# lambdaclass/lambda_elliptic_curves

Measured on AMD Instinct MI355X. Metric: NTT elems/sec (Stark252 radix-2, 2^24, forward, bit-exact vs CPU: see 'bit_exact') [+ MSM G1 point-adds/sec under 'msm'], higher is better.
Workload: dtype u32x8 (256-bit Montgomery, 32-bit limbs)

## Files before the change

lambda_elliptic_curves_amd/csrc/ntt256.hip:

```cpp
#include <stdlib.h>
#include <vector>
#include "internal.h"
#include "ntt_kernels.cuh"
#include "pass_run.h"

namespace lw {

template <class Fn>
static int with_field(int field, Fn f) {
    if (field == LW_FIELD_STARK252) return f(Stark252{});
    if (field == LW_FIELD_BLS12_381_FR) return f(Fr381{});
    set_error("field %d has no 256-bit NTT", field);
    return LW_ERR_BAD_ARG;
}

template <class F>
static Fe<F> host_root_of_unity(uint32_t order, bool inverse) {
    if (order == 0) return Fe<F>::one();
    Fe<F> g;
    for (int i = 0; i < F::N; i++) g.v[i] = F::root(i);
    g = fe_to_mont<F>(g);
    for (uint32_t i = 0; i < F::TWO_ADICITY - order; i++) g = fe_sqr<F>(g);
    if (inverse) g = fe_inv<F>(g);
    return g;
}

template <class F>
static int upload_power_tables(const Fe<F> &base, uint32_t hbits, uint64_t hi_count, DeviceBuf &lo, DeviceBuf &hi,
                               const Fe<F> *hi_scale = nullptr) {
    const uint64_t lo_count = 1ull << hbits;
    std::vector<uint32_t> hl(lo_count * 8), hh(hi_count * 8);
    Fe<F> acc = Fe<F>::one();
    for (uint64_t i = 0; i < lo_count; i++) {
        for (int k = 0; k < 8; k++) hl[i * 8 + k] = acc.v[k];
        acc = fe_mul<F>(acc, base);
    }
    Fe<F> step = acc;
    acc = hi_scale ? *hi_scale : Fe<F>::one();
    for (uint64_t i = 0; i < hi_count; i++) {
        for (int k = 0; k < 8; k++) hh[i * 8 + k] = acc.v[k];
        acc = fe_mul<F>(acc, step);
    }
    if (lo.ensure(lo_count * 32) || hi.ensure(hi_count * 32)) return LW_ERR_ALLOC;
    LW_HIP_CHECK(hipMemcpy(lo.p, hl.data(), lo_count * 32, hipMemcpyHostToDevice), LW_ERR_LAUNCH);
    LW_HIP_CHECK(hipMemcpy(hi.p, hh.data(), hi_count * 32, hipMemcpyHostToDevice), LW_ERR_LAUNCH);
    return LW_OK;
}

template <class F>
static int ensure_twiddles(Context &c, int field, lw_dir_t dir, uint32_t log2n, hipStream_t stream) {
    TwiddleTable &t = c.tw[field][dir];
    DeviceBuf lo, hi;
    const int rc = ensure_twiddle_table(c, t, log2n, F::TWO_ADICITY, 32, stream, [&](uint32_t L) {
        const uint32_t bits = L - 1, hbits = (bits + 1) / 2;
        const uint64_t count = 1ull << bits;
        const int urc = upload_power_tables<F>(host_root_of_unity<F>(L, dir == LW_DIR_INVERSE), hbits, 1ull << (bits - hbits), lo, hi);
        if (urc) return urc;
        hipLaunchKernelGGL((twiddle_fill_kernel<F>), dim3((uint32_t)((count + 255) / 256)), dim3(256), 0, stream, (uint4 *)t.buf.p,
                           (const uint4 *)lo.p, (const uint4 *)hi.p, bits, hbits, count);
        return (int)LW_OK;
    });
    lo.release();
    hi.release();
    return rc;
}

template <class F>
static void launch_pass(bool last, dim3 grid, hipStream_t stream, const NttPassParams &p) {
    const bool extra = p.cos_in || p.cos_out || p.scale;
    bool wl = last && p.r >= 6;
    uint32_t ws = 0;
    for (uint32_t st = 0; st < p.nsteps && wl; st++)
        if ((1u << (p.r + p.logC - p.k[st])) != (uint32_t)NTT_THREADS) wl = false;
    if (wl)
        for (uint32_t st = 1; st < p.nsteps; st++)
            if (p.k[st] == p.k[st - 1] && (1u << (p.r - p.k[st])) <= 64u) ws |= 1u << st;
    NttPassParams q = p;
    q.wave_sync = ws;
#define LW_LAUNCH_PASS(LASTV, EXTRAV)                                                                                          \
    do {                                                                                                                       \
        if (fx == 8 && wl) hipLaunchKernelGGL((ntt_pass_kernel<F, LASTV, EXTRAV, LASTV, FXOK ? 8 : 0>), grid, dim3(NTT_THREADS), 0, stream, q);   \
        else if (fx == 8) hipLaunchKernelGGL((ntt_pass_kernel<F, LASTV, EXTRAV, false, FXOK ? 8 : 0>), grid, dim3(NTT_THREADS), 0, stream, q);   \
        else if (fx == 6 && !wl) hipLaunchKernelGGL((ntt_pass_kernel<F, LASTV, EXTRAV, false, FXOK ? 6 : 0>), grid, dim3(NTT_THREADS), 0, stream, q);   \
        else if (fx == 7 && !wl) hipLaunchKernelGGL((ntt_pass_kernel<F, LASTV, EXTRAV, false, FXOK ? 7 : 0>), grid, dim3(NTT_THREADS), 0, stream, q);   \
        else if (wl) hipLaunchKernelGGL((ntt_pass_kernel<F, LASTV, EXTRAV, LASTV>), grid, dim3(NTT_THREADS), 0, stream, q);  \
        else hipLaunchKernelGGL((ntt_pass_kernel<F, LASTV, EXTRAV, false>), grid, dim3(NTT_THREADS), 0, stream, q);      \
    } while (0)
    constexpr bool FXOK = NTT_TILE == 2048 && NTT_THREADS == 512;
    int fx = 0;
    if (FXOK && p.r == 8 && p.logC == 3 && p.nsteps == 4 && p.k[0] == 2 && p.k[1] == 2 && p.k[2] == 2 && p.k[3] == 2) fx = 8;
    if (FXOK && p.r == 7 && p.logC == 4 && p.nsteps == 4 && p.k[0] == 2 && p.k[1] == 2 && p.k[2] == 2 && p.k[3] == 1) fx = 7;
    if (FXOK && p.r == 6 && p.logC == 5 && p.nsteps == 3 && p.k[0] == 2 && p.k[1] == 2 && p.k[2] == 2) fx = 6;
    if (last) {
        if (extra) LW_LAUNCH_PASS(true, true);
        else LW_LAUNCH_PASS(true, false);
    } else {
        if (extra) LW_LAUNCH_PASS(false, true);
        else LW_LAUNCH_PASS(false, false);
    }
#undef LW_LAUNCH_PASS
}

template <class F>
static int power_tables(Context &c, int field, int slot, const uint32_t *base_words, bool invert, uint32_t hbits,
                        uint32_t hi_bits, hipStream_t stream, const uint4 **lo, const uint4 **hi, bool fold_ninv = false) {
    CosetCache &cc = c.coset[slot];
    bool hit = cc.valid && cc.field == field && cc.hbits == hbits && cc.hi_bits == hi_bits && cc.inverse == invert &&
               cc.fold_ninv == fold_ninv;
    for (int i = 0; i < 8 && hit; i++) hit = cc.words[i] == base_words[i];
    if (!hit) {
        Fe<F> b;
        for (int i = 0; i < 8; i++) b.v[i] = base_words[i];
        if (b.is_zero()) {
            set_error("coset offset is zero");
            return LW_ERR_INV_ZERO;
        }
        if (invert) b = fe_inv<F>(b);
        const uint64_t lo_count = 1ull << hbits, hi_count = 1ull << hi_bits;
        if (cc.lo.ensure(lo_count * 32) || cc.hi.ensure(hi_count * 32)) return LW_ERR_ALLOC;
        FeWords8 bw{}, sw{};
        for (int i = 0; i < 8; i++) bw.w[i] = b.v[i];
        if (fold_ninv) {
            const Fe<F> ninv = fe_inv<F>(fe_from_u64<F>(1ull << (hbits + hi_bits)));
            for (int i = 0; i < 8; i++) sw.w[i] = ninv.v[i];
        }
        hipLaunchKernelGGL((power_tables_kernel<F>), dim3((uint32_t)((lo_count + hi_count + 255) / 256)), dim3(256), 0, stream, (uint4 *)cc.lo.p,
                           (uint4 *)cc.hi.p, bw, hbits, hi_count, sw, fold_ninv ? 1 : 0);
        LW_HIP_CHECK(hipGetLastError(), LW_ERR_LAUNCH);
        cc.valid = true;
        cc.fold_ninv = fold_ninv;
        cc.field = field;
        cc.hbits = hbits;
        cc.hi_bits = hi_bits;
        cc.inverse = invert;
        for (int i = 0; i < 8; i++) cc.words[i] = base_words[i];
    }
    *lo = (const uint4 *)cc.lo.p;
    *hi = (const uint4 *)cc.hi.p;
    return LW_OK;
}

template <class F>
static int ntt256_run(Context &c, int field, lw_dir_t dir, const void *d_in, void *d_out, uint32_t log2n,
                      uint32_t batch, uint64_t stride, const uint32_t *coset_words, hipStream_t stream, uint32_t in_log2) {
    const uint64_t n = 1ull << log2n;
    if (stride == 0) stride = n;
    uint32_t skip = 0;
    if (dir == LW_DIR_FORWARD && in_log2 >= 1 && in_log2 < log2n) skip = log2n - in_log2;
    const uint64_t in_mask = skip ? ((1ull << in_log2) - 1) : ~0ull;
    if (log2n == 0) {
        if (d_in != d_out)
            LW_HIP_CHECK(hipMemcpy2DAsync(d_out, stride * 32, d_in, stride * 32, 32, batch, hipMemcpyDeviceToDevice, stream),
                         LW_ERR_LAUNCH);
        return LW_OK;
    }
    int rc = ensure_twiddles<F>(c, field, dir, log2n, stream);
    if (rc) return rc;
    const uint4 *tw = (const uint4 *)c.tw[field][dir].buf.p;

    const NttPlan pl = plan_passes(log2n, log2n, skip, NTT_TILE_LOG, NTT_KMAX, true);
    if ((pl.npass > 1 || d_in == d_out) && c.scratch.ensure((size_t)n * batch * 32)) return LW_ERR_ALLOC;
    c.timings.scratch_bytes = c.scratch.bytes;

    const uint4 *cos_lo = nullptr, *cos_hi = nullptr;
    const uint32_t cos_hbits = (log2n + 1) / 2;
    if (coset_words) {
        const bool inv = dir == LW_DIR_INVERSE;
        rc = power_tables<F>(c, field, inv ? 1 : 0, coset_words, inv, cos_hbits, log2n - cos_hbits, stream, &cos_lo, &cos_hi, inv);
        if (rc) return rc;
    }
    return run_passes(c, schedule_passes(pl, false, d_in == d_out), log2n, d_in, skip ? (1ull << in_log2) : stride, d_out, stride, batch,
                      c.scratch.p, 32, stream, [&](const PassStep &st, const void *in, void *out, uint64_t in_stride, uint64_t out_stride, dim3 grid) {
        NttPassParams p{};
        p.tw = tw;
        p.lazy_in = (F::LAZY && st.i > 0) ? 1 : 0;
        p.in_mask = st.first ? in_mask : ~0ull;
        p.cos_lo = cos_lo;
        p.cos_hi = cos_hi;
        p.cos_hbits = cos_hbits;
        p.cos_in = (coset_words && dir == LW_DIR_FORWARD && st.first) ? 1 : 0;
        p.cos_out = (coset_words && dir == LW_DIR_INVERSE && st.last) ? 1 : 0;
        p.L = log2n;
        p.s0 = st.s0;
        p.r = st.r;
        p.logC = st.logC;
        p.nsteps = st.nsteps;
        for (uint32_t q = 0; q < p.nsteps; q++) p.k[q] = st.k[q];
        p.in = (const uint4 *)in;
        p.in_batch_stride = in_stride;
        p.out = (uint4 *)out;
        p.out_batch_stride = out_stride;
        if (st.last && dir == LW_DIR_INVERSE) {
            Fe<F> ninv = fe_inv<F>(fe_from_u64<F>(n));
            p.scale = 1;
            for (int k = 0; k < 8; k++) p.sc[k] = ninv.v[k];
        }
        launch_pass<F>(st.last, grid, stream, p);
        return st.last ? "ntt_pass_kernel<last>" : "ntt_pass_kernel";
    });
}

int ntt256_power_tables(Context &c, int field, int slot, const uint32_t *base_words, bool invert, uint32_t hbits,
                        uint32_t hi_bits, hipStream_t stream, const uint4 **lo, const uint4 **hi) {
    return with_field(field, [&](auto f) { return power_tables<decltype(f)>(c, field, slot, base_words, invert, hbits, hi_bits, stream, lo, hi); });
}
int ntt256_root_words(int field, uint32_t order, bool inverse, uint32_t *words) {
    return with_field(field, [&](auto f) {
        const auto w = host_root_of_unity<decltype(f)>(order, inverse);
        for (int i = 0; i < 8; i++) words[i] = w.v[i];
        return (int)LW_OK;
    });
}
int ntt256_inv_u64_words(int field, uint64_t v, uint32_t *words) {
    return with_field(field, [&](auto f) {
        using F = decltype(f);
        const Fe<F> w = fe_inv<F>(fe_from_u64<F>(v));
        for (int i = 0; i < 8; i++) words[i] = w.v[i];
        return (int)LW_OK;
    });
}
const uint4 *ntt256_twiddle_table(Context &c, int field, lw_dir_t dir, uint32_t log2n, hipStream_t stream, int *rc) {
    *rc = with_field(field, [&](auto f) { return ensure_twiddles<decltype(f)>(c, field, dir, log2n, stream); });
    return *rc ? nullptr : (const uint4 *)c.tw[field][dir].buf.p;
}

template <class F>
__global__ void powers_export_kernel(uint4 *out, const uint4 *lo, const uint4 *hi, uint32_t bitrev, uint32_t hbits, uint64_t count) {
    const uint64_t i = (uint64_t)blockIdx.x * blockDim.x + threadIdx.x;
    if (i >= count) return;
    const uint64_t e = bitrev ? bitrev_bits((uint32_t)i, bitrev) : i;
    const Fe<F> x = fe_mul<F>(tw_load<F>(lo, e & ((1ull << hbits) - 1)), tw_load<F>(hi, e >> hbits));
    uint4 q0, q1;
    pack_mem<F>(x, q0, q1);
    out[2 * i] = q0;
    out[2 * i + 1] = q1;
}
template <class F>
static int gen_powers_t(uint32_t order, uint64_t count, uint32_t bitrev, bool inverse, const uint32_t *scale_words, void *d_out,
                        hipStream_t stream) {
    uint32_t bits = 0;
    while ((1ull << bits) < count) bits++;
    const uint32_t hbits = (bits + 1) / 2;
    Fe<F> w = host_root_of_unity<F>(order, inverse), sc;
    if (scale_words)
        for (int i = 0; i < 8; i++) sc.v[i] = scale_words[i];
    DeviceBuf lo, hi;
    int rc = upload_power_tables<F>(w, hbits, 1ull << (bits - hbits), lo, hi, scale_words ? &sc : nullptr);
    if (rc == LW_OK) {
        hipLaunchKernelGGL((powers_export_kernel<F>), dim3((uint32_t)((count + 255) / 256)), dim3(256), 0, stream, (uint4 *)d_out,
                           (const uint4 *)lo.p, (const uint4 *)hi.p, bitrev, hbits, count);
        if (hipGetLastError() != hipSuccess || hipStreamSynchronize(stream) != hipSuccess) {
            set_error("power table kernel failed");
            rc = LW_ERR_LAUNCH;
        }
    }
    lo.release();
    hi.release();
    return rc;
}
int ntt256_gen_powers(int field, uint32_t order, uint64_t count, uint32_t bitrev, bool inverse, const uint32_t *scale_words, void *d_out,
                      hipStream_t stream) {
    return with_field(field, [&](auto f) { return gen_powers_t<decltype(f)>(order, count, bitrev, inverse, scale_words, d_out, stream); });
}

int ntt256_device(Context &c, int field, lw_dir_t dir, const void *d_in, void *d_out, uint32_t log2n, uint32_t batch,
                  uint64_t stride, const uint32_t *coset_words, hipStream_t stream, uint32_t in_log2) {
    return with_field(field, [&](auto f) {
        return ntt256_run<decltype(f)>(c, field, dir, d_in, d_out, log2n, batch, stride, coset_words, stream, in_log2);
    });
}

}
```

lambda_elliptic_curves_amd/csrc/ntt_kernels.cuh:

```cuda
#pragma once
#include "field.cuh"
#include "ntt_bound_plan.h"

namespace lw {

constexpr int NTT_TILE_LOG = 11;
constexpr int NTT_TILE = 1 << NTT_TILE_LOG;
constexpr int NTT_THREADS = 512;
constexpr int NTT_KMAX = 2;
constexpr int NTT_LTW = 256;

struct NttPassParams {
    const uint4 *in;
    uint4 *out;
    const uint4 *tw;
    uint64_t in_batch_stride;
    uint64_t out_batch_stride;
    uint32_t L;
    uint32_t s0;
    uint32_t r;
    uint32_t logC;
    uint32_t nsteps;
    uint32_t k[8];
    const uint4 *cos_lo, *cos_hi;
    uint32_t cos_hbits;
    uint32_t cos_in;
    uint32_t cos_out;
    uint64_t in_mask;
    uint32_t lazy_in;
    uint32_t wave_sync;
    uint32_t scale;
    uint32_t sc[8];
};

__device__ __forceinline__ uint32_t bitrev_bits(uint32_t x, uint32_t bits) {
    return bits ? (__brev(x) >> (32 - bits)) : 0u;
}

template <class F>
__device__ __forceinline__ Fe<F> tw_load(const uint4 *tw, uint64_t g) {
    uint4 a = tw[2 * g], b = tw[2 * g + 1];
    Fe<F> r;
    r.v[0] = a.x; r.v[1] = a.y; r.v[2] = a.z; r.v[3] = a.w;
    r.v[4] = b.x; r.v[5] = b.y; r.v[6] = b.z; r.v[7] = b.w;
    return r;
}
template <class F>
__device__ __forceinline__ Fe<F> tw_load_uniform(const uint4 *tw, uint64_t g) {
    typedef const __attribute__((address_space(4))) uint32_t *const_words;
    const_words w = (const_words)(uintptr_t)(tw + 2 * g);
    Fe<F> r;
#pragma unroll
    for (int i = 0; i < 8; i++) r.v[i] = w[i];
    return r;
}
template <class F>
__device__ __forceinline__ void tw_store(uint4 *tw, uint64_t g, const Fe<F> &x) {
    tw[2 * g] = make_uint4(x.v[0], x.v[1], x.v[2], x.v[3]);
    tw[2 * g + 1] = make_uint4(x.v[4], x.v[5], x.v[6], x.v[7]);
}

template <class F>
__device__ __forceinline__ Fe<F> unpack_mem(uint4 q0, uint4 q1) {
    Fe<F> r;
    r.v[6] = q0.x; r.v[7] = q0.y; r.v[4] = q0.z; r.v[5] = q0.w;
    r.v[2] = q1.x; r.v[3] = q1.y; r.v[0] = q1.z; r.v[1] = q1.w;
    return r;
}
template <class F>
__device__ __forceinline__ void pack_mem(const Fe<F> &a, uint4 &q0, uint4 &q1) {
    q0 = make_uint4(a.v[6], a.v[7], a.v[4], a.v[5]);
    q1 = make_uint4(a.v[2], a.v[3], a.v[0], a.v[1]);
}

template <bool WL>
__device__ __forceinline__ uint32_t lds_slot(uint32_t m, uint32_t c, uint32_t r, uint32_t logC) {
    if (!WL) return (m << logC) | c;
    const uint32_t sw = r >= 4 ? ((5u * ((m >> 4) & 3u)) ^ ((c & 7u) << 1)) : 0u;
    return (c << r) | (m ^ sw);
}
__device__ __forceinline__ void lds_wave_sync() {
    __builtin_amdgcn_fence(__ATOMIC_RELEASE, "wavefront");
    __builtin_amdgcn_wave_barrier();
    __builtin_amdgcn_fence(__ATOMIC_ACQUIRE, "wavefront");
}

struct NttItemGeo {
    uint32_t c, mbase, m_high, sh;
    uint32_t hi_c;
    uint64_t gbase;
};
template <int K, bool LAST, bool WL, int FX>
__device__ __forceinline__ NttItemGeo ntt_item_geo(const NttPassParams &p, uint32_t w, uint32_t step, uint32_t t0, uint64_t base,
                                                   uint32_t hi_uniform, uint32_t hi_low) {
    const uint32_t r = FX ? (uint32_t)FX : p.r, logC = FX ? (uint32_t)(NTT_TILE_LOG - FX) : p.logC, L = p.L;
    NttItemGeo g;
    g.sh = r - t0 - K;
    uint32_t mr;
    if ((LAST && step == 0) || (WL && (LAST || step > 0))) {
        mr = w & ((1u << (r - K)) - 1);
        g.c = w >> (r - K);
    } else {
        g.c = w & ((1u << logC) - 1);
        mr = w >> logC;
    }
    const uint32_t m_low = mr & ((1u << g.sh) - 1);
    g.m_high = mr >> g.sh;
    g.mbase = (g.m_high << (g.sh + K)) | m_low;
    g.hi_c = hi_uniform;
    g.gbase = base;
    if (LAST) {
        g.hi_c = (bitrev_bits(g.c, logC) << (L - r - logC)) | hi_low;
        g.gbase = (uint64_t)g.hi_c << r;
    }
    return g;
}

__device__ __forceinline__ void ntt_tw_stage_load(const NttPassParams &p, uint32_t r, uint32_t hi_uniform, uint4 &tq0, uint4 &tq1) {
    const uint32_t ti = threadIdx.x;
    if (ti + 1 < (1u << r)) {
        const uint32_t t = 31 - __clz(ti + 1), xg = ti + 1 - (1u << t);
        const uint64_t g = ((uint64_t)hi_uniform << t) | xg;
        tq0 = p.tw[2 * g];
        tq1 = p.tw[2 * g + 1];
    }
}
__device__ __forceinline__ void ntt_tw_stage_store(uint4 (*ltw)[NTT_LTW], uint32_t r, const uint4 &tq0, const uint4 &tq1) {
    const uint32_t ti = threadIdx.x;
    if (ti + 1 < (1u << r)) {
        ltw[0][ti] = tq0;
        ltw[1][ti] = tq1;
    }
}

template <class F, int K, bool LAST, bool EXTRA>
__device__ __forceinline__ void ntt_load_global(const NttPassParams &p, const NttItemGeo &g, const uint4 *gin, uint32_t lgS, Fe<F> *x) {
    constexpr int E = 1 << K;
#pragma unroll
    for (int j = 0; j < E; j++) {
        const uint32_t m = g.mbase | ((uint32_t)j << g.sh);
        const uint64_t e = (LAST ? (g.gbase + m) : (g.gbase + ((uint64_t)m << lgS) + g.c)) & p.in_mask;
        x[j] = unpack_mem<F>(gin[2 * e], gin[2 * e + 1]);
    }
    if (EXTRA && p.cos_in) {
#pragma unroll
        for (int j = 0; j < E; j++) {
            const uint32_t m = g.mbase | ((uint32_t)j << g.sh);
            const uint64_t e = (LAST ? (g.gbase + m) : (g.gbase + ((uint64_t)m << lgS) + g.c)) & p.in_mask;
            Fe<F> pw = fe_mul<F>(tw_load<F>(p.cos_lo, e & ((1ull << p.cos_hbits) - 1)), tw_load<F>(p.cos_hi, e >> p.cos_hbits));
            x[j] = fe_mul<F>(x[j], pw);
        }
    }
}

template <class F, bool LAST, bool WL>
__device__ __forceinline__ Fe<F> ntt_fetch_tw(const NttPassParams &p, const NttItemGeo &g, uint4 (*ltw)[NTT_LTW], uint32_t t0, int q) {
    const int u = 31 - __builtin_clz(q + 1), jt = q + 1 - (1 << u);
    Fe<F> tw;
    if (LAST || WL) {
        const uint64_t gt = ((uint64_t)g.hi_c << (t0 + u)) | ((uint64_t)g.m_high << u);
        tw = tw_load<F>(p.tw, gt | (uint32_t)jt);
    } else {
        const uint32_t li = (1u << (t0 + u)) - 1 + ((g.m_high << u) | (uint32_t)jt);
        uint4 a = ltw[0][li], b = ltw[1][li];
        tw.v[0] = a.x; tw.v[1] = a.y; tw.v[2] = a.z; tw.v[3] = a.w;
        tw.v[4] = b.x; tw.v[5] = b.y; tw.v[6] = b.z; tw.v[7] = b.w;
    }
    return tw;
}

template <class F, int K, bool LAST, bool WL, bool PF, bool UNI = false, int FX = 0>
__device__ __forceinline__ void ntt_butterflies(const NttPassParams &p, const NttItemGeo &g, uint4 (*ltw)[NTT_LTW], uint32_t t0, bool first,
                                                Fe<F> *x) {
    constexpr int E = 1 << K;
    static_assert(!UNI || (!LAST && !WL), "wave-uniform twiddles: plain non-last passes only");
    const uint32_t m_high = UNI ? (uint32_t)__builtin_amdgcn_readfirstlane((int)g.m_high) : g.m_high;
    constexpr bool OFFSET = F::LAZY && FX != 0;
    constexpr NttBoundPlan BP = ntt_bound_plan(FX ? FX : 1);
    if constexpr (OFFSET) {
        if (first) {
            if (p.lazy_in) {
#pragma unroll
                for (int j = 0; j < E / 2; j++) x[j] = fe_sub_qp(x[j]);
            }
#pragma unroll
            for (int j = 0; j < E / 2; j++) x[j] = fe_add_cp<BP.c>(x[j]);
        }
    } else if (F::LAZY && first && p.lazy_in) {
#pragma unroll
        for (int j = 0; j < E / 2; j++) x[j] = fe_reduce_full(x[j]);
    }

    auto fetch_tw = [&](int q) -> Fe<F> { return ntt_fetch_tw<F, LAST, WL>(p, g, ltw, t0, q); };
    Fe<F> tw_next, tw_uni[E - 1];
    if (UNI) {
#pragma unroll
        for (int q = 0; q < E - 1; q++) {
            const int u = 31 - __builtin_clz(q + 1), jt = q + 1 - (1 << u);
            tw_uni[q] = tw_load_uniform<F>(p.tw, ((uint64_t)g.hi_c << (t0 + u)) | ((uint64_t)m_high << u) | (uint32_t)jt);
        }
    } else if (PF) {
        tw_next = fetch_tw(0);
    }
#pragma unroll
    for (int q = 0; q < E - 1; q++) {
        const int u = 31 - __builtin_clz(q + 1), jt = q + 1 - (1 << u);
        const int half = 1 << (K - 1 - u);
        const Fe<F> tw = UNI ? tw_uni[q] : PF ? tw_next : fetch_tw(q);
        if (!UNI && PF && q + 1 < E - 1) tw_next = fetch_tw(q + 1);
        const bool unit = (jt == 0) && (g.hi_c == 0) && (m_high == 0);
        const bool free_stage = OFFSET && t0 + (uint32_t)u < (uint32_t)BP.nfree;
#pragma unroll
        for (int jl = 0; jl < half; jl++) {
            const int j = (jt << (K - u)) | jl;
            if (F::LAZY) {
                Fe<F> wb = unit ? fe_reduce_full(x[j + half]) : UNI ? fe_mul_lazy_uniform<F>(tw, x[j + half]) : fe_mul_lazy<F>(tw, x[j + half]);
                if (free_stage) fe_butterfly_raw<F, true>(x[j], wb);
                else fe_butterfly_raw<F, false>(x[j], wb);
                x[j + half] = wb;
            } else {
                Fe<F> wb = unit ? x[j + half] : fe_mul<F>(tw, x[j + half]);
                Fe<F> a = x[j];
                x[j] = fe_add<F>(a, wb);
                x[j + half] = fe_sub<F>(a, wb);
            }
            __builtin_amdgcn_sched_barrier(0);
        }
    }
}

template <class F, int K, bool LAST, bool EXTRA, int FX>
__device__ __forceinline__ void ntt_finish(const NttPassParams &p, const NttItemGeo &g, Fe<F> *x) {
    constexpr int E = 1 << K;
    const uint32_t r = FX ? (uint32_t)FX : p.r, logC = FX ? (uint32_t)(NTT_TILE_LOG - FX) : p.logC, L = p.L;
    if (EXTRA && LAST && p.cos_out) {
#pragma unroll
        for (int j = 0; j < E; j++) {
            const uint32_t m = g.mbase | ((uint32_t)j << g.sh);
            const uint64_t i_nat = ((uint64_t)bitrev_bits(m, r) << (L - r)) + ((uint64_t)blockIdx.x << logC) + g.c;
            Fe<F> pw = fe_mul<F>(tw_load<F>(p.cos_lo, i_nat & ((1ull << p.cos_hbits) - 1)), tw_load<F>(p.cos_hi, i_nat >> p.cos_hbits));
            if (F::LAZY) x[j] = fe_cond_sub_kp<F, 0>(fe_mul_lazy<F>(pw, x[j]));
            else x[j] = fe_mul<F>(x[j], pw);
        }
    } else if (EXTRA && p.scale) {
        Fe<F> sc;
#pragma unroll
        for (int i = 0; i < 8; i++) sc.v[i] = p.sc[i];
#pragma unroll
        for (int j = 0; j < E; j++) {
            if (F::LAZY) x[j] = fe_cond_sub_kp<F, 0>(fe_mul_lazy<F>(sc, x[j]));
            else x[j] = fe_mul<F>(x[j], sc);
        }
    } else if (F::LAZY && LAST) {
#pragma unroll
        for (int j = 0; j < E; j++) x[j] = fe_reduce_full(x[j]);
    }
}

template <class F, int K>
__device__ __forceinline__ void ntt_store_global(const NttItemGeo &g, uint4 *gout, uint32_t lgS, const Fe<F> *x) {
#pragma unroll
    for (int j = 0; j < (1 << K); j++) {
        const uint32_t m = g.mbase | ((uint32_t)j << g.sh);
        const uint64_t e = g.gbase + ((uint64_t)m << lgS) + g.c;
        uint4 q0, q1;
        pack_mem<F>(x[j], q0, q1);
        gout[2 * e] = q0;
        gout[2 * e + 1] = q1;
    }
}

template <class F, int K, bool LAST, bool EXTRA, bool WL, int FX = 0>
__device__ __forceinline__ void ntt_item(const NttPassParams &p, uint4 (*lds)[NTT_TILE], uint4 (*ltw)[NTT_LTW], const uint4 *gin,
                                         uint4 *gout, uint32_t w, uint32_t step, uint32_t t0, uint64_t base, uint32_t lgS,
                                         uint32_t hi_uniform, uint32_t hi_low, bool last_step, bool stage_tw) {
    constexpr int E = 1 << K;
    const uint32_t r = FX ? (uint32_t)FX : p.r, logC = FX ? (uint32_t)(NTT_TILE_LOG - FX) : p.logC;
    const NttItemGeo g = ntt_item_geo<K, LAST, WL, FX>(p, w, step, t0, base, hi_uniform, hi_low);
    uint4 tq0, tq1;
    if (!LAST && !WL && stage_tw) ntt_tw_stage_load(p, r, hi_uniform, tq0, tq1);
    Fe<F> x[E];
    if (step == 0) {
        ntt_load_global<F, K, LAST, EXTRA>(p, g, gin, lgS, x);
    } else {
#pragma unroll
        for (int j = 0; j < E; j++) {
            const uint32_t idx = lds_slot<WL>(g.mbase | ((uint32_t)j << g.sh), g.c, r, logC);
            x[j] = unpack_mem<F>(lds[0][idx], lds[1][idx ^ (WL ? 1u : 0u)]);
        }
    }
    if (!LAST && !WL && stage_tw) {
        ntt_tw_stage_store(ltw, r, tq0, tq1);
        __syncthreads();
    }
    ntt_butterflies<F, K, LAST, WL, true, false, FX>(p, g, ltw, t0, step == 0, x);
    if (last_step) ntt_finish<F, K, LAST, EXTRA, FX>(p, g, x);
    if (!LAST && last_step) {
        ntt_store_global<F, K>(g, gout, lgS, x);
        return;
    }
#pragma unroll
    for (int j = 0; j < E; j++) {
        const uint32_t idx = lds_slot<WL>(g.mbase | ((uint32_t)j << g.sh), g.c, r, logC);
        pack_mem<F>(x[j], lds[0][idx], lds[1][idx ^ (WL ? 1u : 0u)]);
    }
}

template <bool LAST, int FX>
constexpr bool ntt_one_plane() { return FX && !LAST; }
template <class F, bool LAST, bool EXTRA, int FX>
constexpr int ntt_waves_per_simd() { return ntt_one_plane<LAST, FX>() && F::LAZY && !EXTRA ? 6 : 4; }

template <class F>
__device__ __forceinline__ void ntt_exchange(uint4 *lds, const uint32_t (&so)[4], const uint32_t (&si)[4], Fe<F> *x) {
    uint4 o0[4], o1[4], n0[4];
#pragma unroll
    for (int j = 0; j < 4; j++) pack_mem<F>(x[j], o0[j], o1[j]);
#pragma unroll
    for (int j = 0; j < 4; j++) lds[so[j]] = o0[j];
    __syncthreads();
#pragma unroll
    for (int j = 0; j < 4; j++) n0[j] = lds[si[j]];
    __syncthreads();
#pragma unroll
    for (int j = 0; j < 4; j++) lds[so[j]] = o1[j];
    __syncthreads();
#pragma unroll
    for (int j = 0; j < 4; j++) x[j] = unpack_mem<F>(n0[j], lds[si[j]]);
}

template <int K, int FX>
__device__ __forceinline__ void ntt_item_slots(const NttItemGeo &g, uint32_t *s) {
#pragma unroll
    for (int j = 0; j < (1 << K); j++) s[j] = lds_slot<false>(g.mbase | ((uint32_t)j << g.sh), g.c, FX, NTT_TILE_LOG - FX);
}

template <class F, bool EXTRA, int FX>
__device__ __forceinline__ void ntt_tile_fx(const NttPassParams &p, uint4 *lds, uint4 (*ltw)[NTT_LTW], const uint4 *gin, uint4 *gout,
                                            uint64_t base, uint32_t lgS, uint32_t hi_uniform) {
    constexpr bool PF = ntt_waves_per_simd<F, false, EXTRA, FX>() < 6;
    static_assert(NTT_TILE_LOG - NTT_KMAX == 9 && NTT_THREADS == 512, "wave-uniform twiddles of steps 0 and 1 assume 512 radix-4 items");
    const uint32_t tid = threadIdx.x;
    Fe<F> x[4];
    uint32_t so[4], si[4];

    NttItemGeo g = ntt_item_geo<2, false, false, FX>(p, tid, 0u, 0u, base, hi_uniform, 0u);
    uint4 tq0, tq1;
    ntt_tw_stage_load(p, FX, hi_uniform, tq0, tq1);
    ntt_load_global<F, 2, false, EXTRA>(p, g, gin, lgS, x);
    ntt_tw_stage_store(ltw, FX, tq0, tq1);
    ntt_butterflies<F, 2, false, false, PF, true, FX>(p, g, ltw, 0u, true, x);
    ntt_item_slots<2, FX>(g, so);
#pragma unroll
    for (uint32_t s = 1; s < FX / 2; s++) {
        g = ntt_item_geo<2, false, false, FX>(p, tid, s, 2 * s, base, hi_uniform, 0u);
        ntt_item_slots<2, FX>(g, si);
        ntt_exchange<F>(lds, so, si, x);
        if (s == 1) ntt_butterflies<F, 2, false, false, PF, true, FX>(p, g, ltw, 2 * s, false, x);
        else ntt_butterflies<F, 2, false, false, PF, false, FX>(p, g, ltw, 2 * s, false, x);
#pragma unroll
        for (int j = 0; j < 4; j++) so[j] = si[j];
    }
    if constexpr (FX % 2) {
        const NttItemGeo ga = ntt_item_geo<1, false, false, FX>(p, tid, FX / 2, FX - 1, base, hi_uniform, 0u);
        const NttItemGeo gb = ntt_item_geo<1, false, false, FX>(p, tid + NTT_THREADS, FX / 2, FX - 1, base, hi_uniform, 0u);
        ntt_item_slots<1, FX>(ga, si);
        ntt_item_slots<1, FX>(gb, si + 2);
        ntt_exchange<F>(lds, so, si, x);
        ntt_butterflies<F, 1, false, false, PF, false, FX>(p, ga, ltw, FX - 1, false, x);
        ntt_butterflies<F, 1, false, false, PF, false, FX>(p, gb, ltw, FX - 1, false, x + 2);
        ntt_finish<F, 1, false, EXTRA, FX>(p, ga, x);
        ntt_finish<F, 1, false, EXTRA, FX>(p, gb, x + 2);
        ntt_store_global<F, 1>(ga, gout, lgS, x);
        ntt_store_global<F, 1>(gb, gout, lgS, x + 2);
    } else {
        ntt_finish<F, 2, false, EXTRA, FX>(p, g, x);
        ntt_store_global<F, 2>(g, gout, lgS, x);
    }
}

template <class F, bool LAST, bool EXTRA, bool WL, int FX = 0>
__global__ __launch_bounds__(NTT_THREADS, (ntt_waves_per_simd<F, LAST, EXTRA, FX>())) void ntt_pass_kernel(NttPassParams p) {
    __shared__ uint4 lds[ntt_one_plane<LAST, FX>() ? 1 : 2][NTT_TILE];
    __shared__ uint4 ltw[LAST ? 1 : 2][LAST ? 1 : NTT_LTW];
    const uint32_t tid = threadIdx.x;
    static_assert(!FX || (NTT_TILE == 2048 && NTT_THREADS == 512 && (FX == 8 || FX == 7 || FX == 6)), "FX: 2^8 x 8, 2^7 x 16 or 2^6 x 32 rows x columns");
    static_assert(!WL || LAST, "the column layout is the last pass's");
    const uint32_t r = FX ? (uint32_t)FX : p.r, logC = FX ? (uint32_t)(NTT_TILE_LOG - FX) : p.logC, L = p.L;
    const uint32_t tile_log = r + logC;
    const uint4 *gin = p.in + 2 * (uint64_t)blockIdx.y * p.in_batch_stride;
    uint4 *gout = p.out + 2 * (uint64_t)blockIdx.y * p.out_batch_stride;
    const uint32_t b = blockIdx.x;

    uint64_t base = 0;
    uint32_t lgS = 0, hi_uniform = 0, hi_low = 0;
    if (!LAST) {
        lgS = L - p.s0 - r;
        const uint32_t lo_bits = lgS - logC;
        const uint32_t lo_blk = b & ((1u << lo_bits) - 1);
        hi_uniform = b >> lo_bits;
        base = ((uint64_t)hi_uniform << (L - p.s0)) + ((uint64_t)lo_blk << logC);
    } else {
        hi_low = bitrev_bits(b, L - r - logC);
    }

    if constexpr (ntt_one_plane<LAST, FX>()) {
        ntt_tile_fx<F, EXTRA, FX>(p, lds[0], (uint4 (*)[NTT_LTW])ltw, gin, gout, base, lgS, hi_uniform);
    } else {
    if constexpr (FX) {
#define LW_FX_STEP(S)                                                                                                                  \
    do {                                                                                                                                \
        if (S) {                                                                                                                        \
            if (WL && ((p.wave_sync >> (S)) & 1u)) lds_wave_sync();                                                                     \
            else __syncthreads();                                                                                                       \
        }                                                                                                                               \
        ntt_item<F, 2, LAST, EXTRA, WL, FX>(p, lds, (uint4 (*)[NTT_LTW])ltw, gin, gout, tid, (S), 2u * (S), base, lgS, hi_uniform, hi_low,    \
                                            2 * ((S) + 1) == FX, false);                                                                \
    } while (0)
        LW_FX_STEP(0u);
        LW_FX_STEP(1u);
        LW_FX_STEP(2u);
        if constexpr (FX == 8) LW_FX_STEP(3u);
        if constexpr (FX == 7) {
            __syncthreads();
            ntt_item<F, 1, LAST, EXTRA, WL, FX>(p, lds, (uint4 (*)[NTT_LTW])ltw, gin, gout, tid, 3u, 6u, base, lgS, hi_uniform, hi_low, true, false);
            ntt_item<F, 1, LAST, EXTRA, WL, FX>(p, lds, (uint4 (*)[NTT_LTW])ltw, gin, gout, tid + NTT_THREADS, 3u, 6u, base, lgS, hi_uniform, hi_low, true, false);
        }
#undef LW_FX_STEP
    } else {
    const bool stage_inside = !LAST && !WL && (1u << (tile_log - p.k[0])) >= (uint32_t)NTT_THREADS && (1u << r) <= (uint32_t)NTT_THREADS;
    if (!LAST && !WL && !stage_inside) {
        for (uint32_t i = tid; i + 1 < (1u << r); i += NTT_THREADS) {
            const uint32_t t = 31 - __clz(i + 1), x = i + 1 - (1u << t);
            const uint64_t g = ((uint64_t)hi_uniform << t) | x;
            ltw[0][i] = p.tw[2 * g];
            ltw[1][i] = p.tw[2 * g + 1];
        }
        __syncthreads();
    }
    uint32_t t0 = 0;
    for (uint32_t step = 0; step < p.nsteps; step++) {
        const uint32_t k = p.k[step];
        const uint32_t nitems = 1u << (tile_log - k);
        const bool last_step = (step + 1 == p.nsteps);
        if (step) {
            if (WL && ((p.wave_sync >> step) & 1u)) lds_wave_sync();
            else __syncthreads();
        }
        for (uint32_t w = tid; w < nitems; w += NTT_THREADS) {
            if (NTT_KMAX >= 3 && k == 3) ntt_item<F, (NTT_KMAX >= 3 ? 3 : 1), LAST, EXTRA, WL>(p, lds, (uint4 (*)[NTT_LTW])ltw, gin, gout, w, step, t0, base, lgS, hi_uniform, hi_low, last_step, stage_inside && step == 0 && w == tid);
            else if (k == 2) ntt_item<F, 2, LAST, EXTRA, WL>(p, lds, (uint4 (*)[NTT_LTW])ltw, gin, gout, w, step, t0, base, lgS, hi_uniform, hi_low, last_step, stage_inside && step == 0 && w == tid);
            else ntt_item<F, 1, LAST, EXTRA, WL>(p, lds, (uint4 (*)[NTT_LTW])ltw, gin, gout, w, step, t0, base, lgS, hi_uniform, hi_low, last_step, stage_inside && step == 0 && w == tid);
        }
        t0 += k;
    }
    }
    if constexpr (!LAST) return;
    __syncthreads();

    auto write_one = [&](uint32_t f) {
        const uint32_t e = f >> 1, plane = f & 1;
        const uint32_t c = e & ((1u << logC) - 1);
        const uint32_t m = e >> logC;
        const uint64_t g = ((uint64_t)bitrev_bits(m, r) << (L - r)) + ((uint64_t)b << logC) + c;
        gout[2 * g + plane] = lds[plane][lds_slot<WL>(m, c, r, logC) ^ (WL ? plane : 0u)];
    };
    if constexpr (FX) {
#pragma unroll
        for (int q = 0; q < 2 * NTT_TILE / NTT_THREADS; q++) write_one(tid + (uint32_t)q * NTT_THREADS);
    } else {
        const uint32_t total = 2u << tile_log;
        for (uint32_t f = tid; f < total; f += NTT_THREADS) write_one(f);
    }
    }
}

template <class F>
__global__ void twiddle_fill_kernel(uint4 *tw, const uint4 *lo, const uint4 *hi, uint32_t bits, uint32_t hbits,
                                    uint64_t count) {
    uint64_t g = (uint64_t)blockIdx.x * blockDim.x + threadIdx.x;
    if (g >= count) return;
    uint32_t e = bitrev_bits((uint32_t)g, bits);
    Fe<F> a = tw_load<F>(lo, e & ((1u << hbits) - 1));
    Fe<F> b = tw_load<F>(hi, e >> hbits);
    tw_store<F>(tw, g, fe_mul<F>(a, b));
}

struct FeWords8 {
    uint32_t w[8];
};
template <class F>
__global__ void power_tables_kernel(uint4 *lo, uint4 *hi, FeWords8 base, uint32_t hbits, uint64_t hi_count, FeWords8 scale, int has_scale) {
    const uint64_t t = (uint64_t)blockIdx.x * blockDim.x + threadIdx.x;
    const uint64_t lo_count = 1ull << hbits;
    if (t >= lo_count + hi_count) return;
    const bool is_lo = t < lo_count;
    const uint64_t e = is_lo ? t : ((t - lo_count) << hbits);
    Fe<F> b, r = Fe<F>::one();
#pragma unroll
    for (int k = 0; k < 8; k++) b.v[k] = base.w[k];
    for (int bit = 63 - (e ? __clzll((long long)e) : 63); bit >= 0; bit--) {
        r = fe_sqr<F>(r);
        if ((e >> bit) & 1) r = fe_mul<F>(r, b);
    }
    if (!is_lo && has_scale) {
        Fe<F> sc;
#pragma unroll
        for (int k = 0; k < 8; k++) sc.v[k] = scale.w[k];
        r = fe_mul<F>(r, sc);
    }
    if (is_lo) tw_store<F>(lo, t, r);
    else tw_store<F>(hi, t - lo_count, r);
}

}
```

Measured before the change: 14.20 billion.

## Use half-size tiles with 256 threads for the last wave-local FX8 pass

For lazy-reduction fields, the last radix-2^8 wave-local pass now launches on tiles of 2^10 elements (256 rows by 4 columns) with 256 threads and twice as many blocks. The LDS swizzle and plane XOR are adapted for the 4-column layout. The aim is to cut LDS per block and raise occupancy or spread work over more workgroups. The cost is narrower column segments in the global write-back, which may reduce coalescing, and more blocks to schedule.

```diff
diff --git a/lambda_elliptic_curves_amd/csrc/ntt256.hip b/lambda_elliptic_curves_amd/csrc/ntt256.hip
--- a/lambda_elliptic_curves_amd/csrc/ntt256.hip
+++ b/lambda_elliptic_curves_amd/csrc/ntt256.hip
@@ -79,7 +79,7 @@
     q.wave_sync = ws;
 #define LW_LAUNCH_PASS(LASTV, EXTRAV)                                                                                          \
     do {                                                                                                                       \
-        if (fx == 8 && wl) hipLaunchKernelGGL((ntt_pass_kernel<F, LASTV, EXTRAV, LASTV, FXOK ? 8 : 0>), grid, dim3(NTT_THREADS), 0, stream, q);   \
+        if (fx == 8 && wl) hipLaunchKernelGGL((ntt_pass_kernel<F, LASTV, EXTRAV, LASTV, FXOK ? 8 : 0, (LASTV && FXOK) ? TL8 : NTT_TILE_LOG>), grid8, dim3(ntt_threads(TL8)), 0, stream, q8);   \
         else if (fx == 8) hipLaunchKernelGGL((ntt_pass_kernel<F, LASTV, EXTRAV, false, FXOK ? 8 : 0>), grid, dim3(NTT_THREADS), 0, stream, q);   \
         else if (fx == 6 && !wl) hipLaunchKernelGGL((ntt_pass_kernel<F, LASTV, EXTRAV, false, FXOK ? 6 : 0>), grid, dim3(NTT_THREADS), 0, stream, q);   \
         else if (fx == 7 && !wl) hipLaunchKernelGGL((ntt_pass_kernel<F, LASTV, EXTRAV, false, FXOK ? 7 : 0>), grid, dim3(NTT_THREADS), 0, stream, q);   \
@@ -91,6 +91,10 @@
     if (FXOK && p.r == 8 && p.logC == 3 && p.nsteps == 4 && p.k[0] == 2 && p.k[1] == 2 && p.k[2] == 2 && p.k[3] == 2) fx = 8;
     if (FXOK && p.r == 7 && p.logC == 4 && p.nsteps == 4 && p.k[0] == 2 && p.k[1] == 2 && p.k[2] == 2 && p.k[3] == 1) fx = 7;
     if (FXOK && p.r == 6 && p.logC == 5 && p.nsteps == 3 && p.k[0] == 2 && p.k[1] == 2 && p.k[2] == 2) fx = 6;
+    constexpr int TL8 = F::LAZY ? NTT_HALF_LOG : NTT_TILE_LOG;
+    NttPassParams q8 = q;
+    q8.logC = TL8 - 8;
+    const dim3 grid8(grid.x << (NTT_TILE_LOG - TL8), grid.y);
     if (last) {
         if (extra) LW_LAUNCH_PASS(true, true);
         else LW_LAUNCH_PASS(true, false);
diff --git a/lambda_elliptic_curves_amd/csrc/ntt_kernels.cuh b/lambda_elliptic_curves_amd/csrc/ntt_kernels.cuh
--- a/lambda_elliptic_curves_amd/csrc/ntt_kernels.cuh
+++ b/lambda_elliptic_curves_amd/csrc/ntt_kernels.cuh
@@ -9,6 +9,8 @@
 constexpr int NTT_THREADS = 512;
 constexpr int NTT_KMAX = 2;
 constexpr int NTT_LTW = 256;
+constexpr int NTT_HALF_LOG = 10;
+constexpr int ntt_threads(int TL) { return 1 << (TL - NTT_KMAX); }
 
 struct NttPassParams {
     const uint4 *in;
@@ -73,12 +75,14 @@
     q1 = make_uint4(a.v[2], a.v[3], a.v[0], a.v[1]);
 }
 
-template <bool WL>
+template <bool WL, bool HALF = false>
 __device__ __forceinline__ uint32_t lds_slot(uint32_t m, uint32_t c, uint32_t r, uint32_t logC) {
     if (!WL) return (m << logC) | c;
-    const uint32_t sw = r >= 4 ? ((5u * ((m >> 4) & 3u)) ^ ((c & 7u) << 1)) : 0u;
+    const uint32_t sw = r >= 4 ? ((5u * ((m >> 4) & 3u)) ^ (HALF ? (c & 3u) << 2 : (c & 7u) << 1)) : 0u;
     return (c << r) | (m ^ sw);
 }
+template <bool WL, bool HALF = false>
+constexpr uint32_t lds_plane_xor() { return WL ? (HALF ? 2u : 1u) : 0u; }
 __device__ __forceinline__ void lds_wave_sync() {
     __builtin_amdgcn_fence(__ATOMIC_RELEASE, "wavefront");
     __builtin_amdgcn_wave_barrier();
@@ -90,10 +94,10 @@
     uint32_t hi_c;
     uint64_t gbase;
 };
-template <int K, bool LAST, bool WL, int FX>
+template <int K, bool LAST, bool WL, int FX, int TL = NTT_TILE_LOG>
 __device__ __forceinline__ NttItemGeo ntt_item_geo(const NttPassParams &p, uint32_t w, uint32_t step, uint32_t t0, uint64_t base,
                                                    uint32_t hi_uniform, uint32_t hi_low) {
-    const uint32_t r = FX ? (uint32_t)FX : p.r, logC = FX ? (uint32_t)(NTT_TILE_LOG - FX) : p.logC, L = p.L;
+    const uint32_t r = FX ? (uint32_t)FX : p.r, logC = FX ? (uint32_t)(TL - FX) : p.logC, L = p.L;
     NttItemGeo g;
     g.sh = r - t0 - K;
     uint32_t mr;
@@ -229,10 +233,10 @@
     }
 }
 
-template <class F, int K, bool LAST, bool EXTRA, int FX>
+template <class F, int K, bool LAST, bool EXTRA, int FX, int TL = NTT_TILE_LOG>
 __device__ __forceinline__ void ntt_finish(const NttPassParams &p, const NttItemGeo &g, Fe<F> *x) {
     constexpr int E = 1 << K;
-    const uint32_t r = FX ? (uint32_t)FX : p.r, logC = FX ? (uint32_t)(NTT_TILE_LOG - FX) : p.logC, L = p.L;
+    const uint32_t r = FX ? (uint32_t)FX : p.r, logC = FX ? (uint32_t)(TL - FX) : p.logC, L = p.L;
     if (EXTRA && LAST && p.cos_out) {
 #pragma unroll
         for (int j = 0; j < E; j++) {
@@ -270,13 +274,14 @@
     }
 }
 
-template <class F, int K, bool LAST, bool EXTRA, bool WL, int FX = 0>
-__device__ __forceinline__ void ntt_item(const NttPassParams &p, uint4 (*lds)[NTT_TILE], uint4 (*ltw)[NTT_LTW], const uint4 *gin,
+template <class F, int K, bool LAST, bool EXTRA, bool WL, int FX = 0, int TL = NTT_TILE_LOG>
+__device__ __forceinline__ void ntt_item(const NttPassParams &p, uint4 (*lds)[1 << TL], uint4 (*ltw)[NTT_LTW], const uint4 *gin,
                                          uint4 *gout, uint32_t w, uint32_t step, uint32_t t0, uint64_t base, uint32_t lgS,
                                          uint32_t hi_uniform, uint32_t hi_low, bool last_step, bool stage_tw) {
     constexpr int E = 1 << K;
-    const uint32_t r = FX ? (uint32_t)FX : p.r, logC = FX ? (uint32_t)(NTT_TILE_LOG - FX) : p.logC;
-    const NttItemGeo g = ntt_item_geo<K, LAST, WL, FX>(p, w, step, t0, base, hi_uniform, hi_low);
+    const uint32_t r = FX ? (uint32_t)FX : p.r, logC = FX ? (uint32_t)(TL - FX) : p.logC;
+    constexpr bool HALF = TL == NTT_HALF_LOG;
+    const NttItemGeo g = ntt_item_geo<K, LAST, WL, FX, TL>(p, w, step, t0, base, hi_uniform, hi_low);
     uint4 tq0, tq1;
     if (!LAST && !WL && stage_tw) ntt_tw_stage_load(p, r, hi_uniform, tq0, tq1);
     Fe<F> x[E];
@@ -285,8 +290,8 @@
     } else {
 #pragma unroll
         for (int j = 0; j < E; j++) {
-            const uint32_t idx = lds_slot<WL>(g.mbase | ((uint32_t)j << g.sh), g.c, r, logC);
-            x[j] = unpack_mem<F>(lds[0][idx], lds[1][idx ^ (WL ? 1u : 0u)]);
+            const uint32_t idx = lds_slot<WL, HALF>(g.mbase | ((uint32_t)j << g.sh), g.c, r, logC);
+            x[j] = unpack_mem<F>(lds[0][idx], lds[1][idx ^ lds_plane_xor<WL, HALF>()]);
         }
     }
     if (!LAST && !WL && stage_tw) {
@@ -294,15 +299,15 @@
         __syncthreads();
     }
     ntt_butterflies<F, K, LAST, WL, true, false, FX>(p, g, ltw, t0, step == 0, x);
-    if (last_step) ntt_finish<F, K, LAST, EXTRA, FX>(p, g, x);
+    if (last_step) ntt_finish<F, K, LAST, EXTRA, FX, TL>(p, g, x);
     if (!LAST && last_step) {
         ntt_store_global<F, K>(g, gout, lgS, x);
         return;
     }
 #pragma unroll
     for (int j = 0; j < E; j++) {
-        const uint32_t idx = lds_slot<WL>(g.mbase | ((uint32_t)j << g.sh), g.c, r, logC);
-        pack_mem<F>(x[j], lds[0][idx], lds[1][idx ^ (WL ? 1u : 0u)]);
+        const uint32_t idx = lds_slot<WL, HALF>(g.mbase | ((uint32_t)j << g.sh), g.c, r, logC);
+        pack_mem<F>(x[j], lds[0][idx], lds[1][idx ^ lds_plane_xor<WL, HALF>()]);
     }
 }
 
@@ -379,14 +384,17 @@
     }
 }
 
-template <class F, bool LAST, bool EXTRA, bool WL, int FX = 0>
-__global__ __launch_bounds__(NTT_THREADS, (ntt_waves_per_simd<F, LAST, EXTRA, FX>())) void ntt_pass_kernel(NttPassParams p) {
-    __shared__ uint4 lds[ntt_one_plane<LAST, FX>() ? 1 : 2][NTT_TILE];
+template <class F, bool LAST, bool EXTRA, bool WL, int FX = 0, int TL = NTT_TILE_LOG>
+__global__ __launch_bounds__(ntt_threads(TL), (ntt_waves_per_simd<F, LAST, EXTRA, FX>())) void ntt_pass_kernel(NttPassParams p) {
+    constexpr uint32_t THREADS = ntt_threads(TL);
+    constexpr bool HALF = TL == NTT_HALF_LOG;
+    __shared__ uint4 lds[ntt_one_plane<LAST, FX>() ? 1 : 2][1 << TL];
     __shared__ uint4 ltw[LAST ? 1 : 2][LAST ? 1 : NTT_LTW];
     const uint32_t tid = threadIdx.x;
-    static_assert(!FX || (NTT_TILE == 2048 && NTT_THREADS == 512 && (FX == 8 || FX == 7 || FX == 6)), "FX: 2^8 x 8, 2^7 x 16 or 2^6 x 32 rows x columns");
+    static_assert(!FX || (NTT_TILE == 2048 && NTT_THREADS == 512 && (FX == 8 || FX == 7 || FX == 6)), "FX: 2^8 x 8, 2^7 x 16 or 2^6 x 32 rows x columns (TL = NTT_HALF_LOG: 2^8 x 4, 256 threads)");
+    static_assert(TL == NTT_TILE_LOG || (HALF && FX == 8 && WL && LAST), "half tiles: the last pass, 2^8 rows x 4 columns, wave-local");
     static_assert(!WL || LAST, "the column layout is the last pass's");
-    const uint32_t r = FX ? (uint32_t)FX : p.r, logC = FX ? (uint32_t)(NTT_TILE_LOG - FX) : p.logC, L = p.L;
+    const uint32_t r = FX ? (uint32_t)FX : p.r, logC = FX ? (uint32_t)(TL - FX) : p.logC, L = p.L;
     const uint32_t tile_log = r + logC;
     const uint4 *gin = p.in + 2 * (uint64_t)blockIdx.y * p.in_batch_stride;
     uint4 *gout = p.out + 2 * (uint64_t)blockIdx.y * p.out_batch_stride;
@@ -414,7 +422,7 @@
             if (WL && ((p.wave_sync >> (S)) & 1u)) lds_wave_sync();                                                                     \
             else __syncthreads();                                                                                                       \
         }                                                                                                                               \
-        ntt_item<F, 2, LAST, EXTRA, WL, FX>(p, lds, (uint4 (*)[NTT_LTW])ltw, gin, gout, tid, (S), 2u * (S), base, lgS, hi_uniform, hi_low,    \
+        ntt_item<F, 2, LAST, EXTRA, WL, FX, TL>(p, lds, (uint4 (*)[NTT_LTW])ltw, gin, gout, tid, (S), 2u * (S), base, lgS, hi_uniform, hi_low,    \
                                             2 * ((S) + 1) == FX, false);                                                                \
     } while (0)
         LW_FX_STEP(0u);
@@ -463,11 +471,11 @@
         const uint32_t c = e & ((1u << logC) - 1);
         const uint32_t m = e >> logC;
         const uint64_t g = ((uint64_t)bitrev_bits(m, r) << (L - r)) + ((uint64_t)b << logC) + c;
-        gout[2 * g + plane] = lds[plane][lds_slot<WL>(m, c, r, logC) ^ (WL ? plane : 0u)];
+        gout[2 * g + plane] = lds[plane][lds_slot<WL, HALF>(m, c, r, logC) ^ (plane ? lds_plane_xor<WL, HALF>() : 0u)];
     };
     if constexpr (FX) {
 #pragma unroll
-        for (int q = 0; q < 2 * NTT_TILE / NTT_THREADS; q++) write_one(tid + (uint32_t)q * NTT_THREADS);
+        for (int q = 0; q < (2 << TL) / (int)THREADS; q++) write_one(tid + (uint32_t)q * THREADS);
     } else {
         const uint32_t total = 2u << tile_log;
         for (uint32_t f = tid; f < total; f += NTT_THREADS) write_one(f);
```

Result: no change. 14.33 billion, median of 6 (+0.9%).
